# VisualComputingInstitute/diffusion-e2e-ft

Measured on AMD Instinct MI355X. Metric: images/sec (768x768, 1-step UNet fwd) full path: VAE encode + SD-v2 UNet @t=999 + VAE decode, higher is better.
Workload: dtype f16

## Files before the change

diffusion-e2e-ft_amd/_lib.py:

```python
import ctypes as C
import os

import torch

from . import build as _build

_LIB = None

F32, F16, BF16 = 0, 1, 2
_DT = {torch.float32: F32, torch.float16: F16, torch.bfloat16: BF16}


def dtype_id(dt):
    try:
        return _DT[dt]
    except KeyError:
        raise TypeError("libe2eft supports float32/float16/bfloat16, got %s" % dt)


class ConvDesc(C.Structure):
    _fields_ = [(n, C.c_int32) for n in (
        "dtype", "batch", "hin", "win", "hl", "wl", "c1", "ldx1", "c2", "ldx2", "kh", "kw", "stride", "pad_t", "pad_l",
        "hout", "wout", "cout", "ldo", "ldr", "ldw")] + [("alpha", C.c_float)]

# ... 9 lines not shown
        ("eps", C.c_float)]


class AttnDesc(C.Structure):
    _fields_ = [(n, C.c_int32) for n in ("dtype", "batch", "heads", "nq", "nk_seg", "kv_nseg", "kv_bmod", "ldq", "ldk", "ldv",
                                          "ldo")] + [("scale", C.c_float)]


class NormalEvalDesc(C.Structure):
    _fields_ = [(n, C.c_int32) for n in ("batch", "height", "width", "reserved")] + [
        ("pred_stride", C.c_int64 * 4), ("gt_stride", C.c_int64 * 4), ("mask_stride", C.c_int64 * 3)]


class D2ntDesc(C.Structure):
    _fields_ = [(n, C.c_int32) for n in ("batch", "height", "width", "refine", "out_format")] + [("depth_scale", C.c_float)]


D2NT_F32, D2NT_U16, D2NT_U8 = range(3)


class HypersimDesc(C.Structure):
    _fields_ = [(n, C.c_int32) for n in ("batch", "height", "width", "color_dtype", "distance_dtype", "depth_format")] + [
        ("focal", C.c_double), ("scale_numerator", C.c_double)]


HYPERSIM_DEPTH_U16, HYPERSIM_DEPTH_F32 = range(2)
HYPERSIM_RECORD = 16


class DepthGtDesc(C.Structure):
    _fields_ = ([(n, C.c_int32) for n in ("batch", "h0", "w0", "raw_dtype")] + [("divisor", C.c_double)]
                + [(n, C.c_int32) for n in ("inf_to_zero", "crop_top", "crop_left", "crop_h", "crop_w")] + [("min_depth", C.c_float), ("max_depth", C.c_float)]
                + [(n, C.c_int32) for n in ("win_y0", "win_y1", "win_x0", "win_x1", "use_ext_mask")])


GT_U16, GT_I32, GT_F32 = range(3)


class NormalGtDesc(C.Structure):
    _fields_ = [(n, C.c_int32) for n in ("batch", "height", "width", "raw_dtype")]


NORMAL_GT_U8, NORMAL_GT_F32 = range(2)


class DsineRgbDesc(C.Structure):
    _fields_ = [(n, C.c_int32) for n in ("batch", "height", "width", "out_layout")]


RGB_HWC, RGB_CHW = range(2)
DSINE_RGB_WS_INTS = 6


OPT_PERSISTENT, OPT_PERSISTENT_GRID, OPT_NARROW_CONV, OPT_NARROW_MFMA, OPT_IGEMM_GENERAL_OPERANDS, OPT_IGEMM2_WAVES, OPT_PATCH_CONV, OPT_THIN_INPUT_CONV, OPT_FUSED_NORM, OPT_ATTN_DMA, OPT_UPCONV_PHASES, OPT_PATCH_CONV_2X2, OPT_PERSISTENT_MIN_QROUNDS, OPT_GN_APPLY_ITERS, OPT_F32_SPLIT, OPT_F32_SPLIT_ATTN = range(16)

_P = C.c_void_p
_I = C.c_int32
_L = C.c_int64
_F = C.c_float
_Z = C.c_size_t

SIGNATURES = {
    "e2eft_version": (_I, []),
    "e2eft_last_error": (C.c_char_p, []),
    "e2eft_build_id": (C.c_char_p, []),
    "e2eft_set_option": (_I, [_I, _I]),
    "e2eft_get_option": (_I, [_I]),
    "e2eft_conv2d_fwd": (_I, [C.POINTER(ConvDesc), _P, _P, _P, _P, _P, _P, _P, _P]),
    "e2eft_gemm": (_I, [C.POINTER(GemmDesc), _P, _P, _P, _P, _P, _P]),
    "e2eft_conv2d_fwd_gnstats": (_I, [C.POINTER(ConvDesc), _P, _P, _P, _P, _P, _P, _P, _P, _Z, C.POINTER(C.c_int32), _P]),
    "e2eft_conv2d_splitk_workspace_bytes": (_Z, [C.POINTER(ConvDesc)]),
    "e2eft_conv2d_fwd_splitk": (_I, [C.POINTER(ConvDesc), _P, _P, _P, _P, _P, _P, _P, _P, _Z, _P]),
    "e2eft_gemm_gnstats": (_I, [C.POINTER(GemmDesc), _P, _P, _P, _P, _P, _I, _P, _Z, C.POINTER(C.c_int32), _P]),
    "e2eft_groupnorm_fwd_pre": (_I, [C.POINTER(GroupNormDesc), _P, _P, _P, _P, _P, _P, _I, _P, _I, _P, _Z, _P]),
    "e2eft_groupnorm_coeff_offset": (_Z, [C.POINTER(GroupNormDesc)]),
    "e2eft_groupnorm_fwd_stats": (_I, [C.POINTER(GroupNormDesc), _P, _P, _P, _P, _I, _P, _I, _P, _Z, _P]),
    "e2eft_conv2d_fwd_normed_supported": (_I, [C.POINTER(ConvDesc)]),
    "e2eft_upconv2x_fwd_supported": (_I, [C.POINTER(ConvDesc)]),
    "e2eft_upconv2x_fwd": (_I, [C.POINTER(ConvDesc), _P, _P, _P, _P, _P, _Z, C.POINTER(C.c_int32), _P]),
    "e2eft_groupnorm_fwd_split": (_I, [C.POINTER(GroupNormDesc), _P, _P, _P, _P, _I, _P, _P, _I, _P, _Z, _P]),
    "e2eft_f32_split_weight": (_I, [_P, _L, _I, _P, _P, _P]),
    "e2eft_f32_split2_cat": (_I, [_P, _I, _I, _P, _I, _I, _L, _P, _I, _P, _P]),
    "e2eft_f32_split2": (_I, [_P, _L, _I, _I, _P, _I, _P, _P]),
    "e2eft_f32_split2_cols": (_I, [_P, _I, _I, _P, _I, _I, _L, _P, _I, _P, _P]),
    "e2eft_f32_split_wgrad_finish": (_I, [_P, _P, _P, _L, _I, _I, _P, _P, _P, _P]),
    "e2eft_conv2d_fwd_f32split_supported": (_I, [C.POINTER(ConvDesc)]),
    "e2eft_conv2d_fwd_f32split": (_I, [C.POINTER(ConvDesc), _P, _P, _P, _P, _P, _P, _P, _P, _Z, C.POINTER(C.c_int32), _P]),
    "e2eft_upconv2x_fwd_f32split_supported": (_I, [C.POINTER(ConvDesc)]),
    "e2eft_upconv2x_fwd_f32split": (_I, [C.POINTER(ConvDesc), _P, _P, _P, _P, _P, _P, _P, _Z, C.POINTER(C.c_int32), _P]),
    "e2eft_gemm_f32split_supported": (_I, [C.POINTER(GemmDesc)]),
    "e2eft_attn_f32split_supported": (_I, [C.POINTER(AttnDesc), _I]),
    "e2eft_gemm_f32split": (_I, [C.POINTER(GemmDesc), _P, _P, _P, _P, _P, _P, _P, _P]),
    "e2eft_conv2d_fwd_normed": (_I, [C.POINTER(ConvDesc), _P, _P, _P, _I, _P, _P, _P, _P, _P, _P, _Z, C.POINTER(C.c_int32), _P]),
    "e2eft_groupnorm_workspace_bytes": (_Z, [C.POINTER(GroupNormDesc)]),
    "e2eft_groupnorm_fwd": (_I, [C.POINTER(GroupNormDesc), _P, _P, _P, _P, _P, _P, _Z, _P]),
    "e2eft_layernorm_fwd": (_I, [_I, _L, _I, _I, _I, _F, _P, _P, _P, _P, _P]),
    "e2eft_geglu_fwd": (_I, [_I, _L, _I, _I, _I, _P, _P, _P]),
    "e2eft_softmax_rows": (_I, [_I, _L, _I, _L, _F, _P, _P]),
    "e2eft_softmax_rows_causal": (_I, [_I, _L, _I, _L, _F, _I, _P, _P]),
    "e2eft_attn_fwd": (_I, [C.POINTER(AttnDesc), _P, _P, _P, _P, _P]),
    "e2eft_attn_fwd_lse": (_I, [C.POINTER(AttnDesc), _P, _P, _P, _P, _P, _P]),
    "e2eft_attn512_workspace_bytes": (_Z, [C.POINTER(AttnDesc)]),
    "e2eft_attn512_fwd": (_I, [C.POINTER(AttnDesc), _P, _P, _P, _P, _P, _Z, _P]),
    "e2eft_attn_bwd_workspace_bytes": (_Z, [C.POINTER(AttnDesc)]),
    "e2eft_attn_bwd": (_I, [C.POINTER(AttnDesc), _P, _P, _P, _P, _P, _I, _P, _P, _I, _P, _I, _P, _I, _P, _Z, _P]),
    "e2eft_nchw_to_nhwc": (_I, [_I, _I, _I, _I, _I, _I, _I, _F, _F, _P, _P, _P]),
    "e2eft_nhwc_to_nchw": (_I, [_I, _I, _I, _I, _I, _I, _F, _F, _P, _P, _P]),
# ... 135 lines not shown
```

diffusion-e2e-ft_amd/csrc/api.hip:

```cpp
#include "common.h"
#include <atomic>

namespace e2eft {

static thread_local char g_err[512] = "";

char* err_buf() { return g_err; }

int fail(int code, const char* fmt, ...) {
    va_list ap;
    va_start(ap, fmt);
    vsnprintf(g_err, sizeof(g_err), fmt, ap);
    va_end(ap);
    return code;
}

int check_launch(const char* what) {
    hipError_t e = hipGetLastError();
    if (e != hipSuccess) return fail(E2EFT_ERR_LAUNCH, "%s: launch failed: %s", what, hipGetErrorString(e));
    return E2EFT_OK;
}

static std::atomic<int> g_cus_of_device[64];
int device_cus() {
    int dev = 0;
    if (hipGetDevice(&dev) != hipSuccess || dev < 0 || dev >= 64) return 0;
    int n = g_cus_of_device[dev].load(std::memory_order_relaxed);
    if (n == 0) {
        if (hipDeviceGetAttribute(&n, hipDeviceAttributeMultiprocessorCount, dev) != hipSuccess || n < 8) return 0;
        n &= ~7;
        g_cus_of_device[dev].store(n, std::memory_order_relaxed);
    }
    return n;
}

static thread_local char g_tag[96] = "";
void tag_kernel(const char* fmt, ...) {
    va_list ap;
    va_start(ap, fmt);
    vsnprintf(g_tag, sizeof(g_tag), fmt, ap);
    va_end(ap);
}
const char* last_tag() { return g_tag; }

static std::atomic<int> g_opt[E2EFT_OPT_COUNT] = {{1}, {0}, {1}, {1}, {0}, {0}, {1}, {1}, {1}, {1}, {1}, {1}, {2}, {0}, {1}, {0}};

int option(int key) { return g_opt[key].load(std::memory_order_relaxed); }

}

extern "C" int e2eft_set_option(int32_t key, int32_t value) {
    using namespace e2eft;
    E2EFT_REQUIRE(key >= 0 && key < E2EFT_OPT_COUNT, "set_option: unknown key %d", key);
    bool ok = value == 0 || value == 1;
    if (key == E2EFT_OPT_PERSISTENT_GRID) ok = value == 0 || (value >= 8 && value % 8 == 0 && value <= 4096);
    if (key == E2EFT_OPT_IGEMM2_WAVES) ok = value == 0 || value == 4 || value == 8;
    if (key == E2EFT_OPT_PERSISTENT_MIN_QROUNDS) ok = value >= 1 && value <= 64;
    if (key == E2EFT_OPT_GN_APPLY_ITERS) ok = value >= 0 && value <= 16;
    E2EFT_REQUIRE(ok, "set_option: value %d out of range for key %d", value, key);
    g_opt[key].store(value, std::memory_order_relaxed);
    return E2EFT_OK;
}
extern "C" int e2eft_get_option(int32_t key) { return key >= 0 && key < E2EFT_OPT_COUNT ? e2eft::option(key) : -1; }

extern "C" const char* e2eft_debug_last_kernel(void) { return e2eft::last_tag(); }

extern "C" int e2eft_version(void) { return E2EFT_VERSION; }
#ifndef E2EFT_BUILD_ID
#define E2EFT_BUILD_ID "unstamped"
#endif
static const char k_build_id[] = "E2EFT_BUILD_ID=" E2EFT_BUILD_ID;
extern "C" const char* e2eft_build_id(void) { return k_build_id + 15; }
extern "C" const char* e2eft_last_error(void) { return e2eft::err_buf(); }
```

diffusion-e2e-ft_amd/csrc/norm.hip:

```cpp
#include "common.h"

namespace e2eft {

struct Triple {
    float n, mean, m2;
};
__device__ __forceinline__ Triple merge(const Triple& A, const Triple& B) {
    if (B.n == 0.f) return A;
    if (A.n == 0.f) return B;
    Triple r;
    r.n = A.n + B.n;
    const float delta = B.mean - A.mean;
    const float f = B.n / r.n;
    r.mean = A.mean + delta * f;
    r.m2 = A.m2 + B.m2 + delta * delta * A.n * f;
    return r;
}

struct GnGeom {
    int batch, hw, c1, ldx1, c2, ldx2, C;
    int nchunks, cpb, nchb, pl;
    int nslabs, slab;
};

template <typename T>
__global__ __launch_bounds__(256) void gn_partial_kernel(GnGeom g, const T* __restrict__ x1, const T* __restrict__ x2,
                                                         float* __restrict__ partial ) {
    constexpr int EPC = 16 / (int)sizeof(T);
    __shared__ float sm[256 * 8 * 3];
    const int tid = threadIdx.x;
    const int chl = tid % g.cpb, pl = tid / g.cpb;
    const int ch = blockIdx.z * g.cpb + chl;
    const int b = blockIdx.y;
    const int p0 = blockIdx.x * g.slab;
    const int p1 = min(p0 + g.slab, g.hw);
    const bool active = pl < g.pl;
    const int c = ch * EPC;
    const T* src;
    int ld;
    if (c < g.c1) { src = x1 + c; ld = g.ldx1; } else { src = x2 + (c - g.c1); ld = g.ldx2; }
    float piv[EPC], s[EPC], ss[EPC];
    float n = 0.f;
#pragma unroll
    for (int e = 0; e < EPC; ++e) piv[e] = s[e] = ss[e] = 0.f;
    if (active) {
        for (int pix = p0 + pl; pix < p1; pix += g.pl) {
            Vec16<T> v = ld16(src + ((long)b * g.hw + pix) * ld);
            if (n == 0.f) {
#pragma unroll
                for (int e = 0; e < EPC; ++e) piv[e] = to_f(v.e[e]);
            }
#pragma unroll
            for (int e = 0; e < EPC; ++e) {
                const float d = to_f(v.e[e]) - piv[e];
                s[e] += d;
                ss[e] += d * d;
            }
            n += 1.f;
        }
    }
    if (active) {
#pragma unroll
        for (int e = 0; e < EPC; ++e) {
            float mean = 0.f, m2 = 0.f;
            if (n > 0.f) {
                const float ds = s[e] / n;
                mean = piv[e] + ds;
                m2 = fmaxf(ss[e] - s[e] * ds, 0.f);
            }
            float* o = sm + ((pl * g.cpb + chl) * EPC + e) * 3;
            o[0] = n; o[1] = mean; o[2] = m2;
        }
    }
    __syncthreads();
    const int cblk = g.cpb * EPC;
    for (int cc = tid; cc < cblk; cc += 256) {
        Triple acc = {0.f, 0.f, 0.f};
        for (int q = 0; q < g.pl; ++q) {
            const float* o = sm + (q * cblk + cc) * 3;
            Triple t = {o[0], o[1], o[2]};
            acc = merge(acc, t);
        }
        const int cg = blockIdx.z * cblk + cc;
        float* o = partial + (((long)b * g.nslabs + blockIdx.x) * g.C + cg) * 3;
        o[0] = acc.n; o[1] = acc.mean; o[2] = acc.m2;
    }
}

template <typename T>
__global__ __launch_bounds__(256) void gn_finalize_kernel(int C, int c1, int groups, float eps, const float* __restrict__ pa,
                                                          int nsa, const float* __restrict__ pb, int nsb,
                                                          const T* __restrict__ gamma, float* __restrict__ ad ,
                                                          float* __restrict__ rstd_out ) {
    __shared__ float sm[256 * 3];
    const int grp = blockIdx.x, b = blockIdx.y, tid = threadIdx.x;
    const int cpg = C / groups;
    const int cbeg = grp * cpg, cend = cbeg + cpg;
    const int na = max(0, min(cend, c1) - cbeg);
    const int items_a = na * nsa, items = items_a + (cpg - na) * nsb;
    const int c2 = C - c1;
    int P = 1;
    while (P < cpg && P < 256) P <<= 1;
    const int tx = tid & (P - 1), ty = tid / P, ny = 256 / P;
    Triple acc = {0.f, 0.f, 0.f};
    auto walk = [&](const float* __restrict__ base, const int ns, const int cstride, const int nch) {
        for (int cc = tx; cc < nch; cc += P) {
            const float* o = base + (long)cc * 3;
            const long step = (long)cstride * 3;
            int sl = ty;
            for (; sl + 3 * ny < ns; sl += 4 * ny) {
                const float* q0 = o + sl * step;
                const float* q1 = q0 + ny * step;
                const float* q2 = q1 + ny * step;
                const float* q3 = q2 + ny * step;
                const Triple t0 = {q0[0], q0[1], q0[2]}, t1 = {q1[0], q1[1], q1[2]}, t2 = {q2[0], q2[1], q2[2]}, t3 = {q3[0], q3[1], q3[2]};
                acc = merge(merge(merge(merge(acc, t0), t1), t2), t3);
            }
            for (; sl < ns; sl += ny) {
                const float* q0 = o + sl * step;
                const Triple t0 = {q0[0], q0[1], q0[2]};
                acc = merge(acc, t0);
            }
        }
    };
    if (na > 0) walk(pa + ((long)b * nsa * c1 + cbeg) * 3, nsa, c1, na);
    if (cpg - na > 0) walk(pb + ((long)b * nsb * c2 + (cbeg + na - c1)) * 3, nsb, c2, cpg - na);
    (void)items;
    sm[tid * 3] = acc.n; sm[tid * 3 + 1] = acc.mean; sm[tid * 3 + 2] = acc.m2;
    __syncthreads();
    for (int st = 128; st > 0; st >>= 1) {
        if (tid < st) {
            Triple A = {sm[tid * 3], sm[tid * 3 + 1], sm[tid * 3 + 2]};
            Triple B = {sm[(tid + st) * 3], sm[(tid + st) * 3 + 1], sm[(tid + st) * 3 + 2]};
            Triple r = merge(A, B);
            sm[tid * 3] = r.n; sm[tid * 3 + 1] = r.mean; sm[tid * 3 + 2] = r.m2;
        }
        __syncthreads();
    }
    const float mean = sm[1];
    const float var = sm[2] / sm[0];
    const float rstd = rsqrtf(var + eps);
    if (tid == 0) rstd_out[(long)b * groups + grp] = rstd;
    for (int cc = tid; cc < cpg; cc += 256) {
        const int c = cbeg + cc;
        const float ga = gamma ? to_f(gamma[c]) : 1.f;
        ad[((long)b * C + c) * 2] = rstd * ga;
        ad[((long)b * C + c) * 2 + 1] = mean;
    }
}

template <typename T>
__global__ __launch_bounds__(256) void gn_apply_kernel(GnGeom g, int silu, int ldy, const T* __restrict__ x1,
                                                       const T* __restrict__ x2, const float* __restrict__ ad,
                                                       const T* __restrict__ beta, T* __restrict__ y) {
    constexpr int EPC = 16 / (int)sizeof(T);
    const int tid = threadIdx.x;
    const int chl = tid % g.cpb, pl = tid / g.cpb;
    if (pl >= g.pl) return;
    const int ch = blockIdx.z * g.cpb + chl;
    const int b = blockIdx.y;
    const int p0 = blockIdx.x * g.slab;
    const int p1 = min(p0 + g.slab, g.hw);
    const int c = ch * EPC;
    const T* src;
    int ld;
    if (c < g.c1) { src = x1 + c; ld = g.ldx1; } else { src = x2 + (c - g.c1); ld = g.ldx2; }
    float a[EPC], mu[EPC], be[EPC];
#pragma unroll
    for (int e = 0; e < EPC; ++e) {
        a[e] = ad[((long)b * g.C + c + e) * 2];
        mu[e] = ad[((long)b * g.C + c + e) * 2 + 1];
        be[e] = beta ? to_f(beta[c + e]) : 0.f;
        if constexpr (sizeof(T) == 2) gn_fold(a[e], mu[e], be[e], a[e], be[e]);
    }
    auto one = [&](long row, const Vec16<T>& v) {
        Vec16<T> o;
#pragma unroll
        for (int e = 0; e < EPC; ++e) {
            float t;
            if constexpr (sizeof(T) == 2) {
                t = gn_act_u(__builtin_fmaf(to_f(v.e[e]), a[e], be[e]), silu != 0);
            } else {
                t = fmaf(to_f(v.e[e]) - mu[e], a[e], be[e]);
                if (silu) t = silu_f(t);
            }
            o.e[e] = from_f<T>(t);
        }
        st16(y + row * ldy + c, o);
    };
    int pix = p0 + pl;
    for (; pix + 3 * g.pl < p1; pix += 4 * g.pl) {
        const long row = (long)b * g.hw + pix;
        Vec16<T> v[4];
#pragma unroll
        for (int u = 0; u < 4; ++u) v[u] = ld16(src + (row + (long)u * g.pl) * ld);
#pragma unroll
        for (int u = 0; u < 4; ++u) one(row + (long)u * g.pl, v[u]);
    }
    for (; pix < p1; pix += g.pl) {
        const long row = (long)b * g.hw + pix;
// ... 49 lines not shown
    auto one = [&](long row, const floatx4& v) {
        half4 h0, h1;
#pragma unroll
        for (int e = 0; e < 4; ++e) {
            float t = fmaf(v[e] - mu[e], a[e], be[e]);
            if (silu) t = silu_f(t);
            t = fminf(fmaxf(t * s, -65504.f), 65504.f);
            const f16 q0 = (f16)t;
            h0[e] = q0;
            h1[e] = (f16)(t - (float)q0);
        }
        *reinterpret_cast<half4*>(planes + row * ldp + c) = h0;
        *reinterpret_cast<half4*>(planes + row * ldp + g.C + c) = h1;
    };
    int pix = p0 + pl;
    for (; pix + 3 * g.pl < p1; pix += 4 * g.pl) {
        const long row = (long)b * g.hw + pix;
        floatx4 v[4];
#pragma unroll
        for (int u = 0; u < 4; ++u) v[u] = *reinterpret_cast<const floatx4*>(src + (row + (long)u * g.pl) * g.ldx1);
#pragma unroll
        for (int u = 0; u < 4; ++u) one(row + (long)u * g.pl, v[u]);
    }
    for (; pix < p1; pix += g.pl) {
        const long row = (long)b * g.hw + pix;
        one(row, *reinterpret_cast<const floatx4*>(src + row * g.ldx1));
    }
}

static int gn_geom(const E2eftGroupNormDesc* d, GnGeom& g) {
    const int epc = 16 / (int)dtype_size(d->dtype);
    g.batch = d->batch; g.hw = d->hw; g.c1 = d->c1; g.ldx1 = d->ldx1; g.c2 = d->c2; g.ldx2 = d->ldx2;
    g.C = d->c1 + d->c2;
    g.nchunks = g.C / epc;
    int nb = 1;
    while (g.nchunks % nb != 0 || g.nchunks / nb > 256) ++nb;
    g.nchb = nb;
    g.cpb = g.nchunks / nb;
    g.pl = 256 / g.cpb;
    long ns = ((long)d->hw + (long)g.pl * 16 - 1) / ((long)g.pl * 16);
    if (ns < 1) ns = 1;
    if (ns > 1024) ns = 1024;
    g.slab = (int)((d->hw + ns - 1) / ns);
    g.nslabs = (d->hw + g.slab - 1) / g.slab;
    return 0;
}

static void gn_geom_one(int dtype, int batch, int hw, int c, int ld, GnGeom& g) {
    E2eftGroupNormDesc d1 = {};
    d1.dtype = dtype; d1.batch = batch; d1.hw = hw; d1.c1 = c; d1.ldx1 = ld; d1.c2 = 0; d1.ldx2 = 0;
    gn_geom(&d1, g);
}

template <typename T>
static int gn_run(const E2eftGroupNormDesc* d, const GnGeom& g, const void* x1, const void* x2, const void* gamma,
                  const void* beta, void* y, const float* pre1, int ns1, const float* pre2, int ns2, void* ws, hipStream_t s) {
    float* wsp = (float*)ws;
    GnGeom g1, g2;
    gn_geom_one(d->dtype, d->batch, d->hw, d->c1, d->ldx1, g1);
    const float* pa = pre1;
    int nsa = ns1;
    if (!pa) {
        hipLaunchKernelGGL((gn_partial_kernel<T>), dim3(g1.nslabs, g1.batch, g1.nchb), dim3(256), 0, s, g1, (const T*)x1, (const T*)nullptr, wsp);
        pa = wsp; nsa = g1.nslabs;
    }
    wsp += (size_t)d->batch * g1.nslabs * d->c1 * 3;
    const float* pb = pre2;
    int nsb = ns2;
    if (d->c2 > 0) {
        gn_geom_one(d->dtype, d->batch, d->hw, d->c2, d->ldx2, g2);
        if (!pb) {
            hipLaunchKernelGGL((gn_partial_kernel<T>), dim3(g2.nslabs, g2.batch, g2.nchb), dim3(256), 0, s, g2, (const T*)x2, (const T*)nullptr, wsp);
            pb = wsp; nsb = g2.nslabs;
        }
        wsp += (size_t)d->batch * g2.nslabs * d->c2 * 3;
    } else {
        pb = pa; nsb = 1;
    }
    float* ad = wsp;
    float* rstd = ad + (size_t)d->batch * g.C * 2;
    hipLaunchKernelGGL((gn_finalize_kernel<T>), dim3(d->groups, g.batch), dim3(256), 0, s, g.C, d->c1, d->groups, d->eps, pa, nsa, pb, nsb,
                       (const T*)gamma, ad, rstd);
    if (!y) return check_launch("groupnorm_stats");
    GnGeom ga = g;
    const int it = option(E2EFT_OPT_GN_APPLY_ITERS);
    const long tensor_bytes = (long)d->batch * d->hw * g.C * (long)dtype_size(d->dtype);
    ga.slab = g.pl * 4 * (it > 0 ? it : (tensor_bytes <= (128L << 20) ? 4 : 2));
    ga.nslabs = (d->hw + ga.slab - 1) / ga.slab;
    hipLaunchKernelGGL((gn_apply_kernel<T>), dim3(ga.nslabs, ga.batch, ga.nchb), dim3(256), 0, s, ga, d->silu, d->ldy, (const T*)x1, (const T*)x2, ad, (const T*)beta, (T*)y);
    return check_launch("groupnorm");
}

static size_t gn_ws_bytes(const E2eftGroupNormDesc* d) {
    GnGeom g1, g2;
    gn_geom_one(d->dtype, d->batch, d->hw, d->c1, d->ldx1, g1);
    size_t f = (size_t)d->batch * g1.nslabs * d->c1 * 3;
    if (d->c2 > 0) {
        gn_geom_one(d->dtype, d->batch, d->hw, d->c2, d->ldx2, g2);
        f += (size_t)d->batch * g2.nslabs * d->c2 * 3;
    }
    f += (size_t)d->batch * (d->c1 + d->c2) * 2 + (size_t)d->batch * d->groups;
    return f * sizeof(float);
}

template <typename T, int EPC>
struct GnBwdCoef {
    float a[EPC], mu[EPC], rs[EPC], be[EPC];
};
template <typename T, int EPC>
__device__ __forceinline__ void gn_bwd_load(GnBwdCoef<T, EPC>& k, int b, int c, int C, int groups, const float* __restrict__ ad,
                                            const float* __restrict__ rstd, const T* __restrict__ beta) {
    const int cpg = C / groups;
#pragma unroll
    for (int e = 0; e < EPC; ++e) {
        k.a[e] = ad[((long)b * C + c + e) * 2];
        k.mu[e] = ad[((long)b * C + c + e) * 2 + 1];
        k.rs[e] = rstd[(long)b * groups + (c + e) / cpg];
        k.be[e] = beta ? to_f(beta[c + e]) : 0.f;
    }
}
__device__ __forceinline__ float silu_grad_f(float z) {
    const float sg = __builtin_amdgcn_rcpf(1.f + __expf(-z));
    return sg * (1.f + z * (1.f - sg));
}

template <typename T>
__global__ __launch_bounds__(256) void gn_bwd_partial_kernel(GnGeom g, int groups, int silu, int lddy, const T* __restrict__ x1,
                                                             const T* __restrict__ x2, const T* __restrict__ dy,
                                                             const float* __restrict__ ad, const float* __restrict__ rstd,
                                                             const T* __restrict__ beta, float* __restrict__ part ) {
    constexpr int EPC = 16 / (int)sizeof(T);
    __shared__ float sm[256 * 8 * 2];
    const int tid = threadIdx.x;
// ... 389 lines not shown
    }
    dot = wave_sum(dot);
    if ((tid & 63) == 0) red[tid >> 6] = dot;
    __syncthreads();
    dot = red[0] + red[1] + red[2] + red[3];
    for (int ch = tid; ch < npad / EPC; ch += 256) {
        Vec16<T> pv = ld16(prow + ch * EPC), dv = ld16(drow + ch * EPC), o;
#pragma unroll
        for (int e = 0; e < EPC; ++e)
            o.e[e] = from_f<T>((ch * EPC + e < n) ? to_f(pv.e[e]) * (to_f(dv.e[e]) - dot) * scale : 0.f);
        st16(drow + ch * EPC, o);
    }
}

template <typename T>
__global__ __launch_bounds__(256) void geglu_bwd_kernel(long rows, int c, int ldh, int lddy, int lddh, const T* __restrict__ hbuf,
                                                        const T* __restrict__ dy, T* __restrict__ dh) {
    constexpr int EPC = 16 / (int)sizeof(T);
    const int cch = c / EPC;
    const long total = rows * cch;
    for (long it = (long)blockIdx.x * 256 + threadIdx.x; it < total; it += (long)gridDim.x * 256) {
        const long r = it / cch;
        const int ch = (int)(it - r * cch);
        Vec16<T> a = ld16(hbuf + r * ldh + ch * EPC), gt = ld16(hbuf + r * ldh + c + ch * EPC), d = ld16(dy + r * lddy + ch * EPC), oa, og;
#pragma unroll
        for (int e = 0; e < EPC; ++e) {
            const float g = to_f(gt.e[e]), dd = to_f(d.e[e]);
            const float cdf = 0.5f * (1.0f + erff(g * 0.70710678118654752440f));
            const float pdf = 0.3989422804014327f * __expf(-0.5f * g * g);
            oa.e[e] = from_f<T>(dd * g * cdf);
            og.e[e] = from_f<T>(dd * to_f(a.e[e]) * (cdf + g * pdf));
        }
        st16(dh + r * lddh + ch * EPC, oa);
        st16(dh + r * lddh + c + ch * EPC, og);
    }
}

}

using namespace e2eft;

static int gn_validate(const E2eftGroupNormDesc* d) {
    E2EFT_REQUIRE(d, "groupnorm: null desc");
    E2EFT_REQUIRE(d->dtype >= 0 && d->dtype <= 2, "groupnorm: bad dtype");
    const int epc = 16 / (int)dtype_size(d->dtype);
    const int C = d->c1 + d->c2;
    E2EFT_REQUIRE(d->batch > 0 && d->hw > 0 && d->groups > 0, "groupnorm: geometry");
    E2EFT_REQUIRE(d->c1 > 0 && d->c1 % epc == 0 && d->c2 >= 0 && d->c2 % epc == 0, "groupnorm: channels (%d,%d) must be multiples of %d", d->c1, d->c2, epc);
    E2EFT_REQUIRE(C % d->groups == 0, "groupnorm: %d channels not divisible by %d groups", C, d->groups);
    E2EFT_REQUIRE(d->ldx1 >= d->c1 && d->ldx1 % epc == 0 && d->ldy >= C && d->ldy % epc == 0, "groupnorm: strides");
    E2EFT_REQUIRE(d->c2 == 0 || (d->ldx2 >= d->c2 && d->ldx2 % epc == 0), "groupnorm: ldx2");
    return 0;
}

extern "C" size_t e2eft_groupnorm_workspace_bytes(const E2eftGroupNormDesc* d) {
    if (gn_validate(d)) return 0;
    return gn_ws_bytes(d);
}

extern "C" int e2eft_groupnorm_fwd_pre(const E2eftGroupNormDesc* d, const void* x1, const void* x2, const void* gamma,
                                       const void* beta, void* y, const float* partial1, int32_t nslabs1,
                                       const float* partial2, int32_t nslabs2, void* workspace, size_t ws_bytes, void* stream) {
    if (int e = gn_validate(d)) return e;
    E2EFT_REQUIRE(x1 && y && workspace, "groupnorm: null pointer");
    E2EFT_REQUIRE(d->c2 == 0 || x2, "groupnorm: x2 missing");
    E2EFT_REQUIRE((!partial1 || nslabs1 > 0) && (!partial2 || nslabs2 > 0), "groupnorm: precomputed statistics need a slab count");
    GnGeom g;
    gn_geom(d, g);
    const size_t need = gn_ws_bytes(d);
    if (ws_bytes < need) return fail(E2EFT_ERR_WORKSPACE, "groupnorm: workspace %zu < %zu", ws_bytes, need);
    E2EFT_REQUIRE(g.batch <= 65535 && g.nchb <= 65535, "groupnorm: grid");
    E2EFT_DISPATCH_DTYPE(d->dtype, T, return gn_run<T>(d, g, x1, x2, gamma, beta, y, partial1, nslabs1, d->c2 > 0 ? partial2 : nullptr, nslabs2,
                                                      workspace, (hipStream_t)stream));
    return 0;
}

extern "C" size_t e2eft_groupnorm_coeff_offset(const E2eftGroupNormDesc* d) {
    if (gn_validate(d)) return 0;
    return gn_ws_bytes(d) - ((size_t)d->batch * (d->c1 + d->c2) * 2 + (size_t)d->batch * d->groups) * sizeof(float);
}

extern "C" int e2eft_groupnorm_fwd_stats(const E2eftGroupNormDesc* d, const void* x1, const void* x2, const void* gamma, const float* partial1,
                                         int32_t nslabs1, const float* partial2, int32_t nslabs2, void* workspace, size_t ws_bytes, void* stream) {
    if (int e = gn_validate(d)) return e;
    E2EFT_REQUIRE(x1 && workspace, "groupnorm_stats: null pointer");
    E2EFT_REQUIRE(d->c2 == 0 || x2, "groupnorm_stats: x2 missing");
    E2EFT_REQUIRE((!partial1 || nslabs1 > 0) && (!partial2 || nslabs2 > 0), "groupnorm_stats: precomputed statistics need a slab count");
    GnGeom g;
    gn_geom(d, g);
    const size_t need = gn_ws_bytes(d);
    if (ws_bytes < need) return fail(E2EFT_ERR_WORKSPACE, "groupnorm_stats: workspace %zu < %zu", ws_bytes, need);
    E2EFT_REQUIRE(g.batch <= 65535 && g.nchb <= 65535, "groupnorm_stats: grid");
    E2EFT_DISPATCH_DTYPE(d->dtype, T, return gn_run<T>(d, g, x1, x2, gamma, nullptr, nullptr, partial1, nslabs1, d->c2 > 0 ? partial2 : nullptr, nslabs2,
                                                      workspace, (hipStream_t)stream));
    return 0;
}

extern "C" int e2eft_groupnorm_fwd_split(const E2eftGroupNormDesc* d, const float* x, const float* gamma, const float* beta, void* planes, int32_t ldp, float* scale,
                                         const float* partial1, int32_t nslabs1, void* workspace, size_t ws_bytes, void* stream) {
    E2EFT_REQUIRE(d && d->dtype == E2EFT_F32 && d->c2 == 0, "groupnorm_fwd_split: one fp32 source");
    E2EFT_REQUIRE(planes && ldp >= 2 * d->c1 && ldp % 4 == 0 && ((uintptr_t)planes & 7) == 0 && d->c1 % 4 == 0, "groupnorm_fwd_split: planes ldp=%d", (int)ldp);
    E2EFT_REQUIRE(scale && ((uintptr_t)scale & 3) == 0, "groupnorm_fwd_split: scale workspace");
    const int rc = e2eft_groupnorm_fwd_stats(d, x, nullptr, gamma, partial1, nslabs1, nullptr, 0, workspace, ws_bytes, stream);
    if (rc) return rc;
    hipLaunchKernelGGL(gn_split_scale_kernel, dim3(1), dim3(256), 0, (hipStream_t)stream, d->c1, sqrtf((float)d->hw * (float)(d->c1 / d->groups)), gamma, beta, scale);
    GnGeom g;
// ... 178 lines not shown
```

include/e2eft.h:

```cpp
#ifndef E2EFT_H
#define E2EFT_H

#include <stddef.h>
#include <stdint.h>

#ifdef __cplusplus
extern "C" {
#endif
#pragma GCC visibility push(default)

#define E2EFT_VERSION 119

enum {
    E2EFT_OK = 0,
    E2EFT_ERR_BAD_ARG = 1,
    E2EFT_ERR_WORKSPACE = 2,
    E2EFT_ERR_LAUNCH = 3,
    E2EFT_ERR_UNSUPPORTED = 4,
};

enum { E2EFT_F32 = 0, E2EFT_F16 = 1, E2EFT_BF16 = 2 };

int e2eft_version(void);
const char* e2eft_last_error(void);
const char* e2eft_build_id(void);

enum {
    E2EFT_OPT_PERSISTENT = 0,
    E2EFT_OPT_PERSISTENT_GRID = 1,
    E2EFT_OPT_NARROW_CONV = 2,
    E2EFT_OPT_NARROW_MFMA = 3,
    E2EFT_OPT_IGEMM_GENERAL_OPERANDS = 4,
    E2EFT_OPT_IGEMM2_WAVES = 5,
    E2EFT_OPT_PATCH_CONV = 6,
    E2EFT_OPT_THIN_INPUT_CONV = 7,
    E2EFT_OPT_FUSED_NORM = 8,
    E2EFT_OPT_ATTN_DMA = 9,
    E2EFT_OPT_UPCONV_PHASES = 10,
    E2EFT_OPT_PATCH_CONV_2X2 = 11,
    E2EFT_OPT_PERSISTENT_MIN_QROUNDS = 12,
    E2EFT_OPT_GN_APPLY_ITERS = 13,
    E2EFT_OPT_F32_SPLIT = 14,
    E2EFT_OPT_F32_SPLIT_ATTN = 15,
    E2EFT_OPT_COUNT = 16
};
int e2eft_set_option(int32_t key, int32_t value);
int e2eft_get_option(int32_t key);

typedef struct E2eftConvDesc {
    int32_t dtype;
    int32_t batch, hin, win, hl, wl;
    int32_t c1, ldx1;
    int32_t c2, ldx2;
    int32_t kh, kw, stride;
    int32_t pad_t, pad_l;
    int32_t hout, wout;
    int32_t cout, ldo;
    int32_t ldr;
    int32_t ldw;
    float alpha;
} E2eftConvDesc;

int e2eft_conv2d_fwd(const E2eftConvDesc* d, const void* x1, const void* x2, const void* w,
                     const void* bias ,
                     const void* rowadd ,
                     const void* residual , void* out, void* stream);

typedef struct E2eftGemmDesc {
    int32_t dtype;
    int32_t m, n, k;
    int32_t lda, ldw, ldo, ldr;
    int32_t nzo, nzi;
    int64_t sa_o, sa_i, sw_o, sw_i, so_o, so_i, sr_o, sr_i;
    int32_t bias_along_m;
    float alpha;
} E2eftGemmDesc;

int e2eft_gemm(const E2eftGemmDesc* d, const void* a, const void* w, const void* bias, const void* residual,
               void* out, void* stream);

int e2eft_conv2d_fwd_gnstats(const E2eftConvDesc* d, const void* x1, const void* x2, const void* w, const void* bias,
                             const void* rowadd, const void* residual, void* out, float* gn_partial,
                             size_t gn_partial_bytes, int32_t* slab_rows, void* stream);
int e2eft_conv2d_fwd_normed_supported(const E2eftConvDesc* d);
int e2eft_upconv2x_fwd_supported(const E2eftConvDesc* d);
int e2eft_upconv2x_fwd(const E2eftConvDesc* d, const void* x, const void* w_phase, const void* bias, void* out, float* gn_partial,
                       size_t gn_partial_bytes, int32_t* slab_rows, void* stream);

int e2eft_f32_split2(const float* x, int64_t pixels, int32_t c, int32_t ldx, void* planes, int32_t ldp, float* scale, void* stream);
int e2eft_f32_split_weight(const float* w, int64_t rows, int32_t c, void* w_split, float* scale, void* stream);
int e2eft_f32_split2_cat(const float* x1, int32_t c1, int32_t ldx1, const float* x2, int32_t c2, int32_t ldx2, int64_t pixels, void* planes, int32_t ldp,
                         float* scale, void* stream);
int e2eft_f32_split2_cols(const float* x1, int32_t c1, int32_t ldx1, const float* x2, int32_t c2, int32_t ldx2, int64_t pixels, void* planes, int32_t ldp,
                          float* colscale, void* stream);
int e2eft_f32_split_wgrad_finish(const float* t0, const float* t1, const float* t2, int64_t cout, int32_t taps, int32_t cin, const float* inv_dy, const float* inv_x,
                                 float* out, void* stream);
int e2eft_conv2d_fwd_f32split_supported(const E2eftConvDesc* d);
// ... 240 lines not shown
```

include/e2eft_debug.h:

```cpp
#ifndef E2EFT_DEBUG_H
#define E2EFT_DEBUG_H
#ifdef __cplusplus
extern "C" {
#endif
#pragma GCC visibility push(default)

const char* e2eft_debug_last_kernel(void);
long e2eft_debug_patch_launches(void);
long e2eft_debug_persistent_launches(void);
long e2eft_debug_thin_launches(void);

int e2eft_debug_read_stamps(long long* host, int nworkgroups);
int e2eft_debug_read_stamps_rt(long long* host, int nworkgroups);
int e2eft_debug_read_stamps5(long long* host, int nworkgroups);
void e2eft_debug_set_flags5(int flags);

#pragma GCC visibility pop
#ifdef __cplusplus
}
#endif
#endif
```

Before: 90.17.

## Fuse GroupNorm finalize into apply kernel for small activations

Adds a gn_finalize_apply kernel that merges the per-slab partial statistics for a range of groups and then normalizes a pixel slice in the same launch, replacing the separate finalize and apply kernels. It is used when the activation is small (under 64 MiB streamed) and the per-workgroup statistics fit a budget, and it is enabled by default through a new option. The aim is to remove one kernel launch and a global round trip through the scale/shift buffer per GroupNorm. In exchange, every slice workgroup recomputes the same group statistics, which duplicates reads of the partials. The finalize reduction is also refactored into a helper shared by both paths.

```diff
diff --git a/diffusion-e2e-ft_amd/_lib.py b/diffusion-e2e-ft_amd/_lib.py
--- a/diffusion-e2e-ft_amd/_lib.py
+++ b/diffusion-e2e-ft_amd/_lib.py
@@ -85,7 +85,7 @@
 DSINE_RGB_WS_INTS = 6
 
 
-OPT_PERSISTENT, OPT_PERSISTENT_GRID, OPT_NARROW_CONV, OPT_NARROW_MFMA, OPT_IGEMM_GENERAL_OPERANDS, OPT_IGEMM2_WAVES, OPT_PATCH_CONV, OPT_THIN_INPUT_CONV, OPT_FUSED_NORM, OPT_ATTN_DMA, OPT_UPCONV_PHASES, OPT_PATCH_CONV_2X2, OPT_PERSISTENT_MIN_QROUNDS, OPT_GN_APPLY_ITERS, OPT_F32_SPLIT, OPT_F32_SPLIT_ATTN = range(16)
+OPT_PERSISTENT, OPT_PERSISTENT_GRID, OPT_NARROW_CONV, OPT_NARROW_MFMA, OPT_IGEMM_GENERAL_OPERANDS, OPT_IGEMM2_WAVES, OPT_PATCH_CONV, OPT_THIN_INPUT_CONV, OPT_FUSED_NORM, OPT_ATTN_DMA, OPT_UPCONV_PHASES, OPT_PATCH_CONV_2X2, OPT_PERSISTENT_MIN_QROUNDS, OPT_GN_APPLY_ITERS, OPT_F32_SPLIT, OPT_F32_SPLIT_ATTN, OPT_GN_FUSED_FINALIZE = range(17)
 
 _P = C.c_void_p
 _I = C.c_int32
diff --git a/diffusion-e2e-ft_amd/csrc/api.hip b/diffusion-e2e-ft_amd/csrc/api.hip
--- a/diffusion-e2e-ft_amd/csrc/api.hip
+++ b/diffusion-e2e-ft_amd/csrc/api.hip
@@ -43,7 +43,7 @@
 }
 const char* last_tag() { return g_tag; }
 
-static std::atomic<int> g_opt[E2EFT_OPT_COUNT] = {{1}, {0}, {1}, {1}, {0}, {0}, {1}, {1}, {1}, {1}, {1}, {1}, {2}, {0}, {1}, {0}};
+static std::atomic<int> g_opt[E2EFT_OPT_COUNT] = {{1}, {0}, {1}, {1}, {0}, {0}, {1}, {1}, {1}, {1}, {1}, {1}, {2}, {0}, {1}, {0}, {1}};
 
 int option(int key) { return g_opt[key].load(std::memory_order_relaxed); }
 
diff --git a/diffusion-e2e-ft_amd/csrc/norm.hip b/diffusion-e2e-ft_amd/csrc/norm.hip
--- a/diffusion-e2e-ft_amd/csrc/norm.hip
+++ b/diffusion-e2e-ft_amd/csrc/norm.hip
@@ -1,4 +1,5 @@
 #include "common.h"
+#include <atomic>
 
 namespace e2eft {
 
@@ -87,6 +88,91 @@
     }
 }
 
+template <int G>
+__device__ __forceinline__ void gn_walk(Triple (&acc)[G], const float* const (&base)[G] , const int ns, const int cstride,
+                                        const int nch, const int tx, const int ty, const int P, const int ny) {
+    const long step = (long)cstride * 3;
+    for (int cc = tx; cc < nch; cc += P) {
+        int sl = ty;
+        for (; sl + 3 * ny < ns; sl += 4 * ny) {
+            Triple t[G][4];
+#pragma unroll
+            for (int j = 0; j < G; ++j) {
+                const float* q = base[j] + (long)cc * 3 + sl * step;
+#pragma unroll
+                for (int u = 0; u < 4; ++u) {
+                    t[j][u].n = q[0]; t[j][u].mean = q[1]; t[j][u].m2 = q[2];
+                    q += ny * step;
+                }
+            }
+#pragma unroll
+            for (int j = 0; j < G; ++j) acc[j] = merge(merge(merge(merge(acc[j], t[j][0]), t[j][1]), t[j][2]), t[j][3]);
+        }
+        for (; sl < ns; sl += ny) {
+            Triple t[G];
+#pragma unroll
+            for (int j = 0; j < G; ++j) {
+                const float* q = base[j] + (long)cc * 3 + sl * step;
+                t[j].n = q[0]; t[j].mean = q[1]; t[j].m2 = q[2];
+            }
+#pragma unroll
+            for (int j = 0; j < G; ++j) acc[j] = merge(acc[j], t[j]);
+        }
+    }
+}
+
+__device__ __forceinline__ void gn_merge_groups(float* __restrict__ sm, const int C, const int c1, const int groups, const int b, const int grp0, const int ng,
+                                                const float* __restrict__ pa, const int nsa, const float* __restrict__ pb, const int nsb) {
+    const int tid = threadIdx.x;
+    const int cpg = C / groups;
+    const int c2 = C - c1;
+    int P = 1;
+    while (P < cpg && P < 256) P <<= 1;
+    const int tx = tid & (P - 1), ty = tid / P, ny = 256 / P;
+    auto put = [&](const int j, const Triple& a) {
+        float* o = sm + (j * 256 + tid) * 3;
+        o[0] = a.n; o[1] = a.mean; o[2] = a.m2;
+    };
+    for (int j = 0; j < ng;) {
+        const int cbeg = (grp0 + j) * cpg;
+        if (j + 2 <= ng && (cbeg + 2 * cpg <= c1 || cbeg >= c1)) {
+            const bool first = cbeg < c1;
+            const float* o = first ? pa + ((long)b * nsa * c1 + cbeg) * 3 : pb + ((long)b * nsb * c2 + (cbeg - c1)) * 3;
+            const float* const base[2] = {o, o + cpg * 3};
+            Triple acc[2] = {{0.f, 0.f, 0.f}, {0.f, 0.f, 0.f}};
+            gn_walk<2>(acc, base, first ? nsa : nsb, first ? c1 : c2, cpg, tx, ty, P, ny);
+            put(j, acc[0]);
+            put(j + 1, acc[1]);
+            j += 2;
+        } else {
+            const int na = max(0, min(cbeg + cpg, c1) - cbeg);
+            Triple acc[1] = {{0.f, 0.f, 0.f}};
+            if (na > 0) {
+                const float* const base[1] = {pa + ((long)b * nsa * c1 + cbeg) * 3};
+                gn_walk<1>(acc, base, nsa, c1, na, tx, ty, P, ny);
+            }
+            if (cpg - na > 0) {
+                const float* const base[1] = {pb + ((long)b * nsb * c2 + (cbeg + na - c1)) * 3};
+                gn_walk<1>(acc, base, nsb, c2, cpg - na, tx, ty, P, ny);
+            }
+            put(j, acc[0]);
+            j += 1;
+        }
+    }
+    __syncthreads();
+    for (int st = 128, sh = 7; st > 0; st >>= 1, --sh) {
+        for (int i = tid; i < ng * st; i += 256) {
+            float* lo = sm + ((i >> sh) * 256 + (i & (st - 1))) * 3;
+            const float* hi = lo + st * 3;
+            const Triple A = {lo[0], lo[1], lo[2]};
+            const Triple B = {hi[0], hi[1], hi[2]};
+            const Triple r = merge(A, B);
+            lo[0] = r.n; lo[1] = r.mean; lo[2] = r.m2;
+        }
+        __syncthreads();
+    }
+}
+
 template <typename T>
 __global__ __launch_bounds__(256) void gn_finalize_kernel(int C, int c1, int groups, float eps, const float* __restrict__ pa,
                                                           int nsa, const float* __restrict__ pb, int nsb,
@@ -95,48 +181,8 @@
     __shared__ float sm[256 * 3];
     const int grp = blockIdx.x, b = blockIdx.y, tid = threadIdx.x;
     const int cpg = C / groups;
-    const int cbeg = grp * cpg, cend = cbeg + cpg;
-    const int na = max(0, min(cend, c1) - cbeg);
-    const int items_a = na * nsa, items = items_a + (cpg - na) * nsb;
-    const int c2 = C - c1;
-    int P = 1;
-    while (P < cpg && P < 256) P <<= 1;
-    const int tx = tid & (P - 1), ty = tid / P, ny = 256 / P;
-    Triple acc = {0.f, 0.f, 0.f};
-    auto walk = [&](const float* __restrict__ base, const int ns, const int cstride, const int nch) {
-        for (int cc = tx; cc < nch; cc += P) {
-            const float* o = base + (long)cc * 3;
-            const long step = (long)cstride * 3;
-            int sl = ty;
-            for (; sl + 3 * ny < ns; sl += 4 * ny) {
-                const float* q0 = o + sl * step;
-                const float* q1 = q0 + ny * step;
-                const float* q2 = q1 + ny * step;
-                const float* q3 = q2 + ny * step;
-                const Triple t0 = {q0[0], q0[1], q0[2]}, t1 = {q1[0], q1[1], q1[2]}, t2 = {q2[0], q2[1], q2[2]}, t3 = {q3[0], q3[1], q3[2]};
-                acc = merge(merge(merge(merge(acc, t0), t1), t2), t3);
-            }
-            for (; sl < ns; sl += ny) {
-                const float* q0 = o + sl * step;
-                const Triple t0 = {q0[0], q0[1], q0[2]};
-                acc = merge(acc, t0);
-            }
-        }
-    };
-    if (na > 0) walk(pa + ((long)b * nsa * c1 + cbeg) * 3, nsa, c1, na);
-    if (cpg - na > 0) walk(pb + ((long)b * nsb * c2 + (cbeg + na - c1)) * 3, nsb, c2, cpg - na);
-    (void)items;
-    sm[tid * 3] = acc.n; sm[tid * 3 + 1] = acc.mean; sm[tid * 3 + 2] = acc.m2;
-    __syncthreads();
-    for (int st = 128; st > 0; st >>= 1) {
-        if (tid < st) {
-            Triple A = {sm[tid * 3], sm[tid * 3 + 1], sm[tid * 3 + 2]};
-            Triple B = {sm[(tid + st) * 3], sm[(tid + st) * 3 + 1], sm[(tid + st) * 3 + 2]};
-            Triple r = merge(A, B);
-            sm[tid * 3] = r.n; sm[tid * 3 + 1] = r.mean; sm[tid * 3 + 2] = r.m2;
-        }
-        __syncthreads();
-    }
+    const int cbeg = grp * cpg;
+    gn_merge_groups(sm, C, c1, groups, b, grp, 1, pa, nsa, pb, nsb);
     const float mean = sm[1];
     const float var = sm[2] / sm[0];
     const float rstd = rsqrtf(var + eps);
@@ -146,6 +192,102 @@
         const float ga = gamma ? to_f(gamma[c]) : 1.f;
         ad[((long)b * C + c) * 2] = rstd * ga;
         ad[((long)b * C + c) * 2 + 1] = mean;
+    }
+}
+
+struct GnFaGeom {
+    int batch, hw, c1, ldx1, c2, ldx2, C, groups;
+    int gpw, slice;
+    int nranges, nslices;
+};
+static constexpr int GN_FA_BATCH = 8;
+static constexpr int GN_FA_MAXG = 64;
+
+template <typename T>
+__global__ __launch_bounds__(256) void gn_finalize_apply_kernel(GnFaGeom g, int silu, int ldy, float eps, const float* __restrict__ pa, int nsa,
+                                                                const float* __restrict__ pb, int nsb, const T* __restrict__ x1, const T* __restrict__ x2,
+                                                                const T* __restrict__ gamma, const T* __restrict__ beta, T* __restrict__ y,
+                                                                float* __restrict__ ad , float* __restrict__ rstd_out ) {
+    constexpr int EPC = 16 / (int)sizeof(T);
+    extern __shared__ float gn_fa_sm[];
+    __shared__ float sg[GN_FA_MAXG * 2];
+    const int total = gridDim.x, xcd = blockIdx.x & 7, q8 = total >> 3, r8 = total & 7;
+    const int w = (xcd < r8 ? xcd * (q8 + 1) : r8 * (q8 + 1) + (xcd - r8) * q8) + (blockIdx.x >> 3);
+    const int range = w % g.nranges, zs = (w / g.nranges) % g.nslices;
+    const int tid = threadIdx.x, b = w / (g.nranges * g.nslices);
+    const int cpg = g.C / g.groups;
+    const int grp0 = range * g.gpw;
+    const int ng = min(g.gpw, g.groups - grp0);
+    for (int j0 = 0; j0 < ng; j0 += GN_FA_BATCH) {
+        const int nb = min(GN_FA_BATCH, ng - j0);
+        gn_merge_groups(gn_fa_sm, g.C, g.c1, g.groups, b, grp0 + j0, nb, pa, nsa, pb, nsb);
+        if (tid < nb) {
+            const float* r = gn_fa_sm + tid * 768;
+            const float mean = r[1];
+            const float var = r[2] / r[0];
+            const float rstd = rsqrtf(var + eps);
+            sg[(j0 + tid) * 2] = mean;
+            sg[(j0 + tid) * 2 + 1] = rstd;
+        }
+        __syncthreads();
+    }
+    const int cbeg = grp0 * cpg, nch = ng * cpg;
+    if (zs == 0) {
+        if (tid < ng) rstd_out[(long)b * g.groups + grp0 + tid] = sg[tid * 2 + 1];
+        for (int cc = tid; cc < nch; cc += 256) {
+            const int c = cbeg + cc, j = cc / cpg;
+            const float ga = gamma ? to_f(gamma[c]) : 1.f;
+            ad[((long)b * g.C + c) * 2] = sg[j * 2 + 1] * ga;
+            ad[((long)b * g.C + c) * 2 + 1] = sg[j * 2];
+        }
+    }
+    const int nvec = nch / EPC;
+    const int npl = 256 / nvec;
+    const int chl = tid % nvec, pl = tid / nvec;
+    if (pl >= npl) return;
+    const int p0 = zs * g.slice;
+    const int p1 = min(p0 + g.slice, g.hw);
+    const int c = cbeg + chl * EPC;
+    const T* src;
+    int ld;
+    if (c < g.c1) { src = x1 + c; ld = g.ldx1; } else { src = x2 + (c - g.c1); ld = g.ldx2; }
+    float a[EPC], mu[EPC], be[EPC];
+#pragma unroll
+    for (int e = 0; e < EPC; ++e) {
+        const int j = (chl * EPC + e) / cpg;
+        const float ga = gamma ? to_f(gamma[c + e]) : 1.f;
+        a[e] = sg[j * 2 + 1] * ga;
+        mu[e] = sg[j * 2];
+        be[e] = beta ? to_f(beta[c + e]) : 0.f;
+        if constexpr (sizeof(T) == 2) gn_fold(a[e], mu[e], be[e], a[e], be[e]);
+    }
+    auto one = [&](long row, const Vec16<T>& v) {
+        Vec16<T> o;
+#pragma unroll
+        for (int e = 0; e < EPC; ++e) {
+            float t;
+            if constexpr (sizeof(T) == 2) {
+                t = gn_act_u(__builtin_fmaf(to_f(v.e[e]), a[e], be[e]), silu != 0);
+            } else {
+                t = fmaf(to_f(v.e[e]) - mu[e], a[e], be[e]);
+                if (silu) t = silu_f(t);
+            }
+            o.e[e] = from_f<T>(t);
+        }
+        st16(y + row * ldy + c, o);
+    };
+    int pix = p0 + pl;
+    for (; pix + 3 * npl < p1; pix += 4 * npl) {
+        const long row = (long)b * g.hw + pix;
+        Vec16<T> v[4];
+#pragma unroll
+        for (int u = 0; u < 4; ++u) v[u] = ld16(src + (row + (long)u * npl) * ld);
+#pragma unroll
+        for (int u = 0; u < 4; ++u) one(row + (long)u * npl, v[u]);
+    }
+    for (; pix < p1; pix += npl) {
+        const long row = (long)b * g.hw + pix;
+        one(row, ld16(src + row * ld));
     }
 }
 
@@ -301,6 +443,38 @@
     gn_geom(&d1, g);
 }
 
+static constexpr long GN_FA_WG_STAT_BYTES = 128L << 10;
+static constexpr long GN_FA_STREAM_BYTES = 64L << 20;
+static std::atomic<long> g_gn_fused_launches{0};
+
+static bool gn_fa_plan(const E2eftGroupNormDesc* d, int nsa, int nsb, GnFaGeom& f, dim3& grid, size_t& lds) {
+    const int esize = (int)dtype_size(d->dtype);
+    const int C = d->c1 + d->c2, cpg = C / d->groups;
+    int n = 1;
+    while (n < d->groups && !((n * cpg * esize) % 16 == 0 && n * cpg * esize >= 128)) ++n;
+    const int nvec = n * cpg * esize / 16;
+    if (n > GN_FA_MAXG || nvec > 256) return false;
+    const int slabs = d->c2 > 0 ? (nsa > nsb ? nsa : nsb) : nsa;
+    if ((long)n * cpg * slabs * 12 > GN_FA_WG_STAT_BYTES) return false;
+    if (2L * d->batch * d->hw * C * esize > GN_FA_STREAM_BYTES) return false;
+    const int cus = device_cus();
+    if (cus <= 0) return false;
+    const int nranges = (d->groups + n - 1) / n;
+    const int npl = 256 / nvec;
+    long want = (2L * cus + (long)nranges * d->batch - 1) / ((long)nranges * d->batch);
+    const long most = ((long)d->hw + npl * 4 - 1) / (npl * 4);
+    if (want > most) want = most;
+    if (want < 1) want = 1;
+    const int slice = (int)((d->hw + want - 1) / want);
+    const int nslices = (d->hw + slice - 1) / slice;
+    if ((long)nranges * nslices * d->batch > (1L << 30)) return false;
+    f.batch = d->batch; f.hw = d->hw; f.c1 = d->c1; f.ldx1 = d->ldx1; f.c2 = d->c2; f.ldx2 = d->ldx2; f.C = C; f.groups = d->groups;
+    f.gpw = n; f.slice = slice; f.nranges = nranges; f.nslices = nslices;
+    grid = dim3((unsigned)(nranges * nslices * d->batch));
+    lds = (size_t)(n < GN_FA_BATCH ? n : GN_FA_BATCH) * 256 * 3 * sizeof(float);
+    return true;
+}
+
 template <typename T>
 static int gn_run(const E2eftGroupNormDesc* d, const GnGeom& g, const void* x1, const void* x2, const void* gamma,
                   const void* beta, void* y, const float* pre1, int ns1, const float* pre2, int ns2, void* ws, hipStream_t s) {
@@ -328,6 +502,17 @@
     }
     float* ad = wsp;
     float* rstd = ad + (size_t)d->batch * g.C * 2;
+    if (y && option(E2EFT_OPT_GN_FUSED_FINALIZE)) {
+        GnFaGeom f;
+        dim3 grid;
+        size_t lds;
+        if (gn_fa_plan(d, nsa, nsb, f, grid, lds)) {
+            hipLaunchKernelGGL((gn_finalize_apply_kernel<T>), grid, dim3(256), lds, s, f, d->silu, d->ldy, d->eps, pa, nsa, pb, nsb, (const T*)x1, (const T*)x2,
+                               (const T*)gamma, (const T*)beta, (T*)y, ad, rstd);
+            g_gn_fused_launches.fetch_add(1, std::memory_order_relaxed);
+            return check_launch("groupnorm");
+        }
+    }
     hipLaunchKernelGGL((gn_finalize_kernel<T>), dim3(d->groups, g.batch), dim3(256), 0, s, g.C, d->c1, d->groups, d->eps, pa, nsa, pb, nsb,
                        (const T*)gamma, ad, rstd);
     if (!y) return check_launch("groupnorm_stats");
@@ -823,6 +1008,8 @@
     E2EFT_REQUIRE(d->c2 == 0 || (d->ldx2 >= d->c2 && d->ldx2 % epc == 0), "groupnorm: ldx2");
     return 0;
 }
+
+extern "C" long e2eft_debug_gn_fused_launches(void) { return e2eft::g_gn_fused_launches.load(); }
 
 extern "C" size_t e2eft_groupnorm_workspace_bytes(const E2eftGroupNormDesc* d) {
     if (gn_validate(d)) return 0;
diff --git a/include/e2eft.h b/include/e2eft.h
--- a/include/e2eft.h
+++ b/include/e2eft.h
@@ -42,7 +42,8 @@
     E2EFT_OPT_GN_APPLY_ITERS = 13,
     E2EFT_OPT_F32_SPLIT = 14,
     E2EFT_OPT_F32_SPLIT_ATTN = 15,
-    E2EFT_OPT_COUNT = 16
+    E2EFT_OPT_GN_FUSED_FINALIZE = 16,
+    E2EFT_OPT_COUNT = 17
 };
 int e2eft_set_option(int32_t key, int32_t value);
 int e2eft_get_option(int32_t key);
diff --git a/include/e2eft_debug.h b/include/e2eft_debug.h
--- a/include/e2eft_debug.h
+++ b/include/e2eft_debug.h
@@ -9,6 +9,7 @@
 long e2eft_debug_patch_launches(void);
 long e2eft_debug_persistent_launches(void);
 long e2eft_debug_thin_launches(void);
+long e2eft_debug_gn_fused_launches(void);
 
 int e2eft_debug_read_stamps(long long* host, int nworkgroups);
 int e2eft_debug_read_stamps_rt(long long* host, int nworkgroups);
```

Result: no change. 90.27 (median of 6 runs) (+0.1%).
